# privacy-scaling-explorations/snark-verifier

Hardware: AMD Instinct MI355X
Metric: BN254 G1 MSM points/sec at 2^20 (higher is better)
Workload: dtype i32x9 (254-bit Montgomery Fq as 9 x 29-bit limbs on the integer VALU); 1 GPU; BN254 G1 Pippenger MSM, 2^20 random points/scalars per GPU, inputs resident in HBM, affine result (configs[1]); points_per_gpu=1048576, points_per_kernel_launch=1048576, window_bits=default, msms_in_flight=264

## Files before the change

### snark-verifier_amd/csrc/ctx.hpp

```cpp
#pragma once
#include <hip/hip_runtime.h>
#include <stddef.h>
#include <stdint.h>
#include <stdio.h>
#include "../../include/snarkv_amd.h"
#include "curve_consts.h"

#if defined(SNARKV_CURVE_PALLAS)
#define SNARKV_API(name) snarkv_pallas_##name
#define SNARKV_CHUNK_PIPELINE 0
#define SNARKV_API_FLAGS SNARKV_FLAG_VALIDATE
#else
#define SNARKV_API(name) snarkv_##name
#define SNARKV_CHUNK_PIPELINE 1
#define SNARKV_API_FLAGS (SNARKV_FLAG_VALIDATE | SNARKV_FLAG_MONTGOMERY)
#endif

namespace snarkv {

void set_last_error(const char* fmt, ...);

#define SNARKV_HIP(expr)                                                                   \
  do {                                                                                     \
    hipError_t _e = (expr);                                                                \
    if (_e != hipSuccess) {                                                                \
      ::snarkv::set_last_error("%s:%d: %s -> %s", __FILE__, __LINE__, #expr, hipGetErrorString(_e)); \
      return SNARKV_ERR_DEVICE;                                                            \
    }                                                                                      \
  } while (0)

#define SNARKV_TRY(expr)      \
  do {                        \
    int _rc = (expr);         \
    if (_rc < 0) return _rc;  \
  } while (0)

enum Slot {
  SLOT_IN_SCALARS = 0,
  SLOT_IN_POINTS,
  SLOT_IN_OFFSETS,
  SLOT_OUT,
  SLOT_POINTS_MONT,
  SLOT_COUNTS,
  SLOT_OFFSETS,
  SLOT_CURSOR,
  SLOT_BLOCKSUMS,
  SLOT_ENTRIES,
  SLOT_PIECES,
  SLOT_SPLIT_PARTS,
  SLOT_PIECE_HIST,
  SLOT_BUCKETS,
  SLOT_CHUNK_PARTIALS,
  SLOT_WINDOW_SUMS,
  SLOT_TERM_PARTIALS,
  SLOT_FLAGS,
  SLOT_MISC,
  SLOT_SORT_TMP,
  SLOT_SHIFTED,
  SLOT_GLV,
  SLOT_FIX_LISTS,
  SLOT_MISC2,
  SLOT_TERM_CHAIN,
  SLOT_TERM_MAGS,
  SLOT_SPLIT_PARTIALS,
  SLOT_IPA_XI,
  SLOT_IPA_H,
  SLOT_IPA_OUT,
  SLOT_MGPU_GRID,
  SLOT_MGPU_RECV,
  SLOT_COUNT
};

}

struct snarkv_ctx {
  int device;
  hipStream_t stream;
  bool own_stream;
  void* buf[snarkv::SLOT_COUNT];
  size_t cap[snarkv::SLOT_COUNT];
  void* hbuf[SNARKV_HOST_BUFFERS];
  size_t hbuf_cap[SNARKV_HOST_BUFFERS];
  uint32_t flags;
  bool mont;
  bool stage_timing;
  float stage_ms[SNARKV_PIP_STAGES];
  hipEvent_t ev[SNARKV_PIP_STAGES + 1];
  bool ev_ready;
  snarkv_ctx* sub[4];
  hipEvent_t sub_ev[5];
  bool sub_ready;
  hipEvent_t sorted_ev;
  bool sorted_ev_ready;
  int last_split_workers;
  bool throughput_mode;
  int throughput_peers;
  bool is_lane;
  snarkv_ctx* jobs[SNARKV_MANY_MAX_JOBS];
  int njobs;
  int last_many_jobs;
  size_t many_sig;
  hipStream_t copy_stream;
  bool copy_ready;
  hipEvent_t many_ev[2];
  hipEvent_t order_ev;
  bool order_ev_ready;
  hipStream_t hi_stream[2];
  bool hi_ready;
};

struct snarkv_dk {
  int device;
  void* d_prep;
  uint8_t g1[64];
};

struct snarkv_ipa_dk {
  int device;
  uint32_t k;
  void* d_points;
  size_t first;
  size_t count;
};

namespace snarkv {

struct CallFlags {
  snarkv_ctx* c;
  bool saved;
  CallFlags(snarkv_ctx* ctx, uint32_t call_flags) : c(ctx), saved(ctx ? ctx->mont : false) {
    if (c) c->mont = ((c->flags | call_flags) & SNARKV_FLAG_MONTGOMERY) != 0;
  }
  ~CallFlags() {
    if (c) c->mont = saved;
  }
};
#define SNARKV_CALL_FLAGS(ctx, f) ::snarkv::CallFlags _call_flags((ctx), (f))
struct WireFormScope {
  snarkv_ctx* c;
  bool saved;
  explicit WireFormScope(snarkv_ctx* ctx) : c(ctx), saved(ctx ? ctx->mont : false) {
    if (c) c->mont = false;
// ... 50 lines not shown
```

### snark-verifier_amd/csrc/glv.h

```cpp
#pragma once
#include "fq.h"

namespace snarkv {

template <int NA, int NB, int NOUT>
SNARKV_HD void mp_mul(const uint32_t* a, const uint32_t* b, uint32_t* out) {
#pragma unroll
  for (int i = 0; i < NOUT; ++i) out[i] = 0;
#pragma unroll
  for (int i = 0; i < NA; ++i) {
    uint64_t carry = 0;
#pragma unroll
    for (int j = 0; j < NB; ++j) {
      if (i + j < NOUT) {
        uint64_t t = (uint64_t)a[i] * b[j] + out[i + j] + carry;
        out[i + j] = (uint32_t)t;
        carry = t >> 32;
      }
    }
    if (i + NB < NOUT) out[i + NB] = (uint32_t)carry;
  }
}

SNARKV_HD void glv_decompose(const uint32_t k[8], uint32_t out[8]) {
  constexpr uint32_t A1[4] = SNARKV_GLV_A1;
  constexpr uint32_t NB1[4] = SNARKV_GLV_NEG_B1;
  constexpr uint32_t A2[4] = SNARKV_GLV_A2;
  constexpr uint32_t B2[4] = SNARKV_GLV_B2;
  constexpr uint32_t G1[6] = SNARKV_GLV_G1;
  constexpr uint32_t G2[6] = SNARKV_GLV_G2;
  uint32_t a1[4], nb1[4], a2[4], b2[4], g1[6], g2[6];
  for (int i = 0; i < 4; ++i) { a1[i] = A1[i]; nb1[i] = NB1[i]; a2[i] = A2[i]; b2[i] = B2[i]; }
  for (int i = 0; i < 6; ++i) { g1[i] = G1[i]; g2[i] = G2[i]; }

  uint32_t t1[14], t2[14];
  mp_mul<8, 6, 14>(k, g1, t1);
  mp_mul<8, 6, 14>(k, g2, t2);
  uint32_t c1[5], c2[5];
  {
    uint64_t carry = ((uint64_t)t1[8] + 0x80000000u) >> 32;
    for (int i = 0; i < 5; ++i) {
      uint64_t v = (uint64_t)t1[9 + i] + carry;
      c1[i] = (uint32_t)v;
      carry = v >> 32;
    }
    carry = ((uint64_t)t2[8] + 0x80000000u) >> 32;
    for (int i = 0; i < 5; ++i) {
      uint64_t v = (uint64_t)t2[9 + i] + carry;
      c2[i] = (uint32_t)v;
      carry = v >> 32;
    }
  }
  uint32_t p1[5], p2[5], k1[5], k2[5];
  mp_mul<5, 4, 5>(c1, a1, p1);
  mp_mul<5, 4, 5>(c2, a2, p2);
  {
    uint64_t borrow = 0;
    for (int i = 0; i < 5; ++i) {
      uint64_t v = (uint64_t)k[i] - p1[i] - borrow;
      k1[i] = (uint32_t)v;
      borrow = (v >> 32) & 1u;
    }
    borrow = 0;
    for (int i = 0; i < 5; ++i) {
      uint64_t v = (uint64_t)k1[i] - p2[i] - borrow;
      k1[i] = (uint32_t)v;
      borrow = (v >> 32) & 1u;
    }
  }
  mp_mul<5, 4, 5>(c1, nb1, p1);
  mp_mul<5, 4, 5>(c2, b2, p2);
  {
    uint64_t borrow = 0;
    for (int i = 0; i < 5; ++i) {
      uint64_t v = (uint64_t)p1[i] - p2[i] - borrow;
      k2[i] = (uint32_t)v;
      borrow = (v >> 32) & 1u;
    }
  }
  uint32_t* halves[2] = {k1, k2};
  for (int h = 0; h < 2; ++h) {
    uint32_t* v = halves[h];
    uint32_t neg = v[4] >> 31;
    if (neg) {
      uint64_t carry = 1;
      for (int i = 0; i < 5; ++i) {
        uint64_t x = (uint64_t)(~v[i]) + carry;
        v[i] = (uint32_t)x;
        carry = x >> 32;
      }
    }
    for (int i = 0; i < 4; ++i) out[4 * h + i] = v[i];
    out[4 * h + 3] |= neg << 31;
  }
}

}
```

### snark-verifier_amd/csrc/msm_pippenger.hip

```cpp
#include <stdlib.h>
#include <string.h>
#include <algorithm>
#include <mutex>
#include <atomic>
#include "ctx.hpp"
#include "g1_29.h"
#include "fr29.h"
#ifndef SNARKV_GLV
#define SNARKV_GLV 1
#endif
#if SNARKV_GLV
#include "glv.h"
#endif

namespace snarkv {

#ifndef SNARKV_KRUN
#define SNARKV_KRUN 128
#endif
#ifndef SNARKV_KCHUNK
#define SNARKV_KCHUNK 8
#endif
#ifndef SNARKV_TILE_THREADS
#define SNARKV_TILE_THREADS 256
#endif
#ifndef SNARKV_SCATTER_ATTR
#define SNARKV_SCATTER_ATTR __attribute__((amdgpu_waves_per_eu(5)))
#endif
#ifndef SNARKV_L2_THREADS
#define SNARKV_L2_THREADS 512
#endif
#ifndef SNARKV_LEVEL2_ATTR
#define SNARKV_LEVEL2_ATTR
#endif
#ifndef SNARKV_PREP_THREADS
#define SNARKV_PREP_THREADS SNARKV_TILE_THREADS
#endif
#ifndef SNARKV_XCD_TILES
#define SNARKV_XCD_TILES 1
#endif
#ifndef SNARKV_TILE_BASE
#define SNARKV_TILE_BASE 2048
#endif
#ifndef SNARKV_ACC_WAVES
#define SNARKV_ACC_WAVES 3
#endif
#ifndef SNARKV_BPRIO
#define SNARKV_BPRIO 3
#endif
#define SNARKV_RAISE_PRIO() __builtin_amdgcn_s_setprio(SNARKV_BPRIO)

constexpr int kHalves = SNARKV_GLV ? 2 : 1;
constexpr int kDigitWords = SNARKV_GLV ? 4 : 8;
constexpr int kDigitBits = 32 * kDigitWords;
constexpr int kRun = SNARKV_KRUN;
#ifndef SNARKV_KRUN_THROUGHPUT
#define SNARKV_KRUN_THROUGHPUT 128
#endif
constexpr int kRunThroughput = SNARKV_KRUN_THROUGHPUT;
constexpr int kChunk = SNARKV_KCHUNK;
constexpr uint32_t kSortCap = 7168;
constexpr uint32_t kSortTarget = 3072;
constexpr uint32_t kMaxKeys = 16384;

struct PipParams {
  uint32_t n;
  int c;
  int W;
  uint32_t B;
  uint32_t nb;
  int low_bits;
  uint32_t SB;
  uint32_t nkeys;
  uint32_t nblk;
  uint32_t tile;
  uint32_t mstride;
  uint32_t w0;
  uint32_t krun;
  uint32_t wper;
  uint32_t chunk_log2;
  uint32_t mont;
};

__device__ __forceinline__ uint32_t half_bits(const uint32_t (&k)[kDigitWords], int lo, int c) {
  if (lo >= kDigitBits) return 0;
  int word = lo >> 5, sh = lo & 31;
  uint32_t w0 = 0u, w1 = 0u;
#pragma unroll
  for (int i = 0; i < kDigitWords; ++i) {
    w0 = word == i ? k[i] : w0;
    if (i > 0) w1 = word == i - 1 ? k[i] : w1;
  }
  uint64_t v = ((uint64_t)w1 << 32) | w0;
  return (uint32_t)(v >> sh) & ((1u << c) - 1u);
}

template <class F>
__device__ __forceinline__ void for_each_digit(const uint32_t (&k)[kDigitWords], uint32_t sgn, const PipParams& p, F emit) {
  uint32_t carry = 0;
  for (int w = 0; w < p.W; ++w) {
    uint32_t raw = half_bits(k, w * p.c, p.c) + carry;
    uint32_t neg = raw > p.B ? 1u : 0u;
    uint32_t d = neg ? ((1u << p.c) - raw) : raw;
    carry = neg;
    if (d != 0) emit((uint32_t)w * p.SB + ((d - 1) >> p.low_bits), (uint32_t)w * p.B + d - 1, neg ^ sgn);
  }
}
template <class F>
__device__ __forceinline__ void digit_of_window(const uint32_t (&k)[kDigitWords], uint32_t sgn, const PipParams& p, int w,
                                                F emit) {
  uint32_t carry = 0;
  for (int j = w - 1; j >= 0; --j) {
    uint32_t b = half_bits(k, j * p.c, p.c);
    if (b != p.B) {
      carry = b > p.B ? 1u : 0u;
      break;
    }
  }
  uint32_t raw = half_bits(k, w * p.c, p.c) + carry;
  uint32_t neg = raw > p.B ? 1u : 0u;
  uint32_t d = neg ? ((1u << p.c) - raw) : raw;
  if (d != 0) emit((uint32_t)w * p.SB + ((d - 1) >> p.low_bits), (uint32_t)w * p.B + d - 1, neg ^ sgn);
}
__device__ __forceinline__ uint32_t load_digit_words(const uint32_t* src, uint32_t (&k)[kDigitWords]) {
#pragma unroll
  for (int j = 0; j < kDigitWords; ++j) k[j] = src[j];
#if SNARKV_GLV
  uint32_t sgn = k[3] >> 31;
  k[3] &= 0x7FFFFFFFu;
  return sgn;
#else
  return 0u;
#endif
}
__device__ __forceinline__ uint32_t load_digit_source(const uint4* __restrict__ src, size_t v, uint32_t (&k)[kDigitWords]) {
  const uint4* s = src + v * (kDigitWords / 4);
#pragma unroll
  for (int j = 0; j < kDigitWords / 4; ++j) {
    uint4 q = s[j];
    k[4 * j] = q.x;
    k[4 * j + 1] = q.y;
    k[4 * j + 2] = q.z;
    k[4 * j + 3] = q.w;
  }
#if SNARKV_GLV
  uint32_t sgn = k[3] >> 31;
  k[3] &= 0x7FFFFFFFu;
  return sgn;
#else
  return 0u;
#endif
}

__device__ __forceinline__ uint32_t xcd_tile(uint32_t b, uint32_t nblk) {
#if SNARKV_XCD_TILES
  return (nblk & 7u) == 0 ? (b & 7u) * (nblk >> 3) + (b >> 3) : b;
#else
  return b;
#endif
}

__global__ void __launch_bounds__(SNARKV_PREP_THREADS)
    k_prepare(const uint32_t* __restrict__ scalars, const uint32_t* __restrict__ points,
              G1Packed* __restrict__ pts, uint4* __restrict__ glv, PipParams p, uint32_t* __restrict__ M) {
  SNARKV_RAISE_PRIO();
  extern __shared__ uint32_t lds[];
  for (uint32_t k = threadIdx.x; k < p.nkeys; k += blockDim.x) lds[k] = 0u;
  __syncthreads();
  const uint32_t tile = xcd_tile(blockIdx.x, p.nblk);
  uint32_t lo = tile * p.tile;
  uint32_t hi = lo + p.tile < p.n ? lo + p.tile : p.n;
  for (uint32_t i = lo + threadIdx.x; i < hi; i += blockDim.x) {
    const uint4* s = reinterpret_cast<const uint4*>(points + (size_t)i * 16);
    uint32_t w[16];
#pragma unroll
    for (int j = 0; j < 4; ++j) {
      uint4 v = s[j];
      w[4 * j] = v.x;
      w[4 * j + 1] = v.y;
      w[4 * j + 2] = v.z;
      w[4 * j + 3] = v.w;
    }
    G1Affine29 a = g1a29_from_words(w, p.mont != 0);
    bool ident = g1a29_is_identity(a);
    pts[kHalves * (size_t)i] = g1a29_pack(a);
    const uint4* ks = reinterpret_cast<const uint4*>(scalars + (size_t)i * 8);
    uint4 k0 = ks[0], k1 = ks[1];
    uint32_t k[8] = {k0.x, k0.y, k0.z, k0.w, k1.x, k1.y, k1.z, k1.w}, o[8];
    if (p.mont) {
      uint32_t kc[8];
      fr_words_from_mont256(k, kc);
#pragma unroll
      for (int j = 0; j < 8; ++j) k[j] = kc[j];
    }
#if SNARKV_GLV
    constexpr int32_t bl[9] = SNARKV_GLV_BETA29_LIMBS;
    Fq29 beta;
#pragma unroll
    for (int j = 0; j < 9; ++j) beta.v[j] = bl[j];
    a.x = fq29_canon_of_product(fq29_mul(a.x, beta));
    pts[2 * (size_t)i + 1] = g1a29_pack(a);
    glv_decompose(k, o);
#else
#pragma unroll
    for (int j = 0; j < 8; ++j) o[j] = k[j];
#endif
    if (ident) {
#pragma unroll
      for (int j = 0; j < 8; ++j) o[j] = 0;
    }
    glv[2 * (size_t)i] = make_uint4(o[0], o[1], o[2], o[3]);
    glv[2 * (size_t)i + 1] = make_uint4(o[4], o[5], o[6], o[7]);
#pragma unroll
    for (int h = 0; h < kHalves; ++h) {
      uint32_t d[kDigitWords];
      uint32_t sgn = load_digit_words(o + h * kDigitWords, d);
      for_each_digit(d, sgn, p, [&](uint32_t key, uint32_t, uint32_t) { atomicAdd(&lds[key], 1u); });
    }
  }
  __syncthreads();
  for (uint32_t k = threadIdx.x; k < p.nkeys; k += blockDim.x) M[(size_t)k * p.mstride + tile] = lds[k];
  if (blockIdx.x == 0 && p.mstride > p.nblk)
    for (uint32_t k = threadIdx.x; k < p.nkeys; k += blockDim.x) M[(size_t)k * p.mstride + p.nblk] = 0u;
}

constexpr uint32_t kStageScalars = SNARKV_TILE_BASE;
constexpr uint32_t kStageItems = kStageScalars / SNARKV_TILE_THREADS;
static_assert(kStageScalars % SNARKV_TILE_THREADS == 0, "a staged tile gives every lane the same number of scalars");
__global__ void __launch_bounds__(SNARKV_TILE_THREADS) SNARKV_SCATTER_ATTR
    k_sort_scatter_staged(const uint4* __restrict__ glv, PipParams p, const uint32_t* __restrict__ M,
                          uint2* __restrict__ tmp) {
  SNARKV_RAISE_PRIO();
  extern __shared__ uint32_t lds[];
  uint32_t* gbase = lds;
  uint32_t* cnt = lds + p.SB;
  uint32_t* off = lds + 2 * p.SB;
  uint32_t* wsum = lds + 3 * p.SB;
  uint2* stage = reinterpret_cast<uint2*>(lds + 3 * p.SB + 16 + (p.SB & 1u));
  const uint32_t tid = threadIdx.x, lane = tid & 63u, wave = tid >> 6;
  const uint32_t tile = xcd_tile(blockIdx.x, p.nblk);
  const uint32_t lo = tile * kStageScalars;
  const uint32_t hi = lo + kStageScalars < p.n ? lo + kStageScalars : p.n;
  const uint32_t per = (p.SB + SNARKV_TILE_THREADS - 1) / SNARKV_TILE_THREADS;
  for (int w = 0; w < p.W; ++w) {
    for (uint32_t k = tid; k < p.SB; k += blockDim.x) {
      gbase[k] = M[((size_t)w * p.SB + k) * p.mstride + tile];
      cnt[k] = 0u;
    }
    __syncthreads();
    uint32_t ebkt[kStageItems * kHalves], erank[kStageItems * kHalves], eneg = 0u;
#pragma unroll
    for (uint32_t j = 0; j < kStageItems; ++j) {
      const uint32_t i = lo + tid + j * SNARKV_TILE_THREADS;
#pragma unroll
      for (uint32_t h = 0; h < (uint32_t)kHalves; ++h) {
        const uint32_t e = j * kHalves + h;
        ebkt[e] = 0xFFFFFFFFu;
        if (i < hi) {
          uint32_t d[kDigitWords];
          uint32_t sgn = load_digit_source(glv, (size_t)kHalves * i + h, d);
          digit_of_window(d, sgn, p, w, [&](uint32_t key, uint32_t bucket, uint32_t neg) {
            ebkt[e] = bucket - (uint32_t)w * p.B;
            eneg |= neg << e;
            erank[e] = atomicAdd(&cnt[key - (uint32_t)w * p.SB], 1u);
          });
        }
      }
    }
    __syncthreads();
    uint32_t mine = 0;
    for (uint32_t k = tid * per; k < (tid + 1) * per && k < p.SB; ++k) mine += cnt[k];
    uint32_t incl = mine;
#pragma unroll
    for (int d = 1; d < 64; d <<= 1) {
      uint32_t up = __shfl_up(incl, d, 64);
      if ((int)lane >= d) incl += up;
    }
    if (lane == 63) wsum[wave] = incl;
    __syncthreads();
    uint32_t run = incl - mine;
    for (uint32_t q = 0; q < wave; ++q) run += wsum[q];
    for (uint32_t k = tid * per; k < (tid + 1) * per && k < p.SB; ++k) {
      off[k] = run;
      run += cnt[k];
    }
    __syncthreads();
#pragma unroll
    for (uint32_t e = 0; e < kStageItems * kHalves; ++e)
      if (ebkt[e] != 0xFFFFFFFFu) {
        const uint32_t v = kHalves * (lo + tid + (e / kHalves) * SNARKV_TILE_THREADS) + (e % kHalves);
        stage[off[ebkt[e] >> p.low_bits] + erank[e]] = make_uint2(ebkt[e] + (uint32_t)w * p.B, v | (((eneg >> e) & 1u) << 31));
      }
    __syncthreads();
    const uint32_t total = off[p.SB - 1] + cnt[p.SB - 1];
    for (uint32_t idx = tid; idx < total; idx += blockDim.x) {
      const uint2 e = stage[idx];
      const uint32_t key = (e.x - (uint32_t)w * p.B) >> p.low_bits;
      tmp[gbase[key] + (idx - off[key])] = e;
    }
    __syncthreads();
  }
}

__global__ void __launch_bounds__(256) k_scan_local(uint32_t* __restrict__ data, uint32_t* __restrict__ blocksum,
                                                    uint32_t nb) {
  SNARKV_RAISE_PRIO();
  __shared__ uint32_t sh[256];
  uint32_t base = blockIdx.x * 1024 + threadIdx.x * 4;
  uint32_t v[4], s = 0;
#pragma unroll
  for (int j = 0; j < 4; ++j) {
    v[j] = (base + j < nb) ? data[base + j] : 0;
    s += v[j];
  }
  sh[threadIdx.x] = s;
  __syncthreads();
  for (uint32_t off = 1; off < 256; off <<= 1) {
    uint32_t t = (threadIdx.x >= off) ? sh[threadIdx.x - off] : 0;
    __syncthreads();
    sh[threadIdx.x] += t;
    __syncthreads();
  }
  uint32_t excl = sh[threadIdx.x] - s;
#pragma unroll
  for (int j = 0; j < 4; ++j) {
    if (base + j < nb) data[base + j] = excl;
    excl += v[j];
  }
  if (threadIdx.x == 255) blocksum[blockIdx.x] = sh[255];
}

__global__ void __launch_bounds__(1024) k_scan_blocksums(uint32_t* __restrict__ blocksum, uint32_t nblocks,
                                                         uint32_t* __restrict__ total_out) {
  SNARKV_RAISE_PRIO();
  __shared__ uint32_t sh[1024];
  __shared__ uint32_t running;
  if (threadIdx.x == 0) running = 0;
  __syncthreads();
  for (uint32_t base = 0; base < nblocks; base += 1024) {
    uint32_t idx = base + threadIdx.x;
    uint32_t v = idx < nblocks ? blocksum[idx] : 0;
    sh[threadIdx.x] = v;
    __syncthreads();
    for (uint32_t off = 1; off < 1024; off <<= 1) {
      uint32_t t = (threadIdx.x >= off) ? sh[threadIdx.x - off] : 0;
      __syncthreads();
      sh[threadIdx.x] += t;
      __syncthreads();
    }
    uint32_t r0 = running;
    if (idx < nblocks) blocksum[idx] = r0 + sh[threadIdx.x] - v;
    __syncthreads();
    if (threadIdx.x == 1023) running = r0 + sh[1023];
    __syncthreads();
  }
  if (threadIdx.x == 0) *total_out = running;
}

__global__ void __launch_bounds__(256) k_scan_add(uint32_t* __restrict__ data, const uint32_t* __restrict__ blocksum,
                                                  uint32_t nb) {
  SNARKV_RAISE_PRIO();
  uint32_t base = blockIdx.x * 1024 + threadIdx.x * 4;
  uint32_t add = blocksum[blockIdx.x];
#pragma unroll
  for (int j = 0; j < 4; ++j)
    if (base + j < nb) data[base + j] += add;
}

__global__ void __launch_bounds__(SNARKV_L2_THREADS) SNARKV_LEVEL2_ATTR
    k_sort_level2(const uint2* __restrict__ tmp, const uint32_t* __restrict__ M, uint32_t* __restrict__ misc,
                  PipParams p, uint2* __restrict__ entries, uint32_t* __restrict__ counts,
                  uint32_t* __restrict__ offsets) {
// ... 451 lines not shown
                     (uint32_t*)d_out64, partial_out ? 1 : 0, ctx->mont ? 1u : 0u);
  SNARKV_HIP(hipGetLastError());
  return SNARKV_OK;
}

static int default_window_bits(size_t n) {
  int best = 2;
  double best_cost = 0;
  for (int c = 2; c <= 22; ++c) {
    const int W = (kDigitBits + c - 1) / c;
    const int top = kDigitBits - 1 - (W - 1) * c;
    double cost = (double)kHalves * (double)n * W * 10.0 + (double)W * (double)(1u << (c - 1)) * 30.0;
    if (top < c - 3) cost *= 1.6;
    if (c == 2 || cost < best_cost) best = c, best_cost = cost;
  }
  return best;
}

static int balance_window_bits(int c) {
  int W = (kDigitBits + c - 1) / c;
  return (kDigitBits + W - 1) / W;
}

static uint32_t latency_run_length(uint64_t entries) {
  auto waves = [&](uint64_t run) { return (entries + 64 * run - 1) / (64 * run); };
  if (waves(16) <= 4608) return waves(16) >= 2048 ? 16u : 32u;
  if (waves(32) <= 4608) return 32u;
  return (uint32_t)kRun;
}
static_assert(kRun >= 32 && kRun <= (int)kMaxPiece && kRunThroughput >= 16 && kRunThroughput <= (int)kMaxPiece,
              "piece caps fit the schedule's LDS rows");

int launch_msm_pippenger(snarkv_ctx* ctx, const void* d_scalars, const void* d_points, size_t n, int window_bits,
                         void* d_out, bool partial_out, void* d_buckets_out) {
  return launch_msm_pippenger_phases(ctx, ctx->stream, PIP_PHASE_ALL, d_scalars, d_points, n, window_bits, d_out,
                                     partial_out, d_buckets_out, nullptr);
}

int launch_msm_pippenger_phases(snarkv_ctx* ctx, hipStream_t st, int phases, const void* d_scalars, const void* d_points,
                                size_t n, int window_bits, void* d_out, bool partial_out, void* d_buckets_out,
                                void* d_grid) {
  PipParams p;
  p.w0 = 0;
  p.wper = 0;
  p.chunk_log2 = (uint32_t)kLog2Chunk;
  p.mont = ctx->mont ? 1u : 0u;
  p.n = (uint32_t)n;
  p.c = window_bits > 0 ? window_bits : balance_window_bits(default_window_bits(n));
  if (p.c < 2) p.c = 2;
  if (p.c > 22) p.c = 22;
  p.W = (kDigitBits + p.c - 1) / p.c;
  p.B = 1u << (p.c - 1);
  p.nb = (uint32_t)p.W * p.B;
  int high = p.c - 1 > 10 ? p.c - 1 - 10 : 0;
  while (high < p.c - 1 && ((kHalves * n) >> (high + 1)) >= kSortTarget && ((uint64_t)p.W << (high + 1)) <= kMaxKeys) ++high;
  p.low_bits = (p.c - 1) - high;
  p.SB = p.B >> p.low_bits;
  p.nkeys = (uint32_t)p.W * p.SB;
  p.tile = SNARKV_TILE_BASE;
  static_assert(kStageItems * kHalves <= 32, "a staged lane keeps one sign bit per entry in a 32-bit word");
  const size_t lds_staged = ((size_t)3 * p.SB + 16 + (p.SB & 1u)) * 4 + (size_t)kStageScalars * kHalves * 8;
  p.nblk = (uint32_t)((n + p.tile - 1) / p.tile);
  p.mstride = p.nblk | 1u;
  uint64_t max_entries = (uint64_t)kHalves * (uint64_t)n * (uint64_t)p.W;
  if (n == 0 || max_entries >= 0xFFFFFFFFull || n >= 0x40000000ull) {
    set_last_error("pippenger: n=%zu out of range", n);
    return SNARKV_ERR_LENGTH;
  }
  if ((size_t)p.nkeys * 4 > 65536 || lds_staged > 96 * 1024) {
    set_last_error("pippenger: key table too large (nkeys=%u)", p.nkeys);
    return SNARKV_ERR_LENGTH;
  }
  p.krun = ctx->throughput_mode ? (uint32_t)kRunThroughput : latency_run_length(max_entries);
  const uint32_t max_pieces = (uint32_t)std::min<uint64_t>((uint64_t)p.nb + max_entries / p.krun, 0xFFFFFFFFull - 63);
  const uint32_t split_slots = (uint32_t)(max_entries / p.krun) + 1;
  const uint32_t nsb = (p.nb + kSchedBuckets - 1) / kSchedBuckets;
  const uint32_t hcount = sched_rows(p.krun) * nsb;
  const uint32_t hscan_blocks = (hcount + 1023) / 1024;
  uint32_t mcount = p.nkeys * p.mstride;
  uint32_t scan_blocks = (mcount + 1023) / 1024;
  uint32_t chunks_per_window = (p.B + kChunk - 1) / kChunk;
  uint32_t blocks_per_window = (chunks_per_window + 63) / 64;

  void *d_pts, *d_glv, *d_counts, *d_offsets, *d_M, *d_blocksum, *d_entries, *d_tmp, *d_pieces, *d_hist, *d_parts,
      *d_buckets, *d_wave, *d_shift, *d_misc, *d_lists;
  SNARKV_TRY(ctx_reserve(ctx, SLOT_POINTS_MONT, kHalves * n * sizeof(G1Packed), &d_pts));
  SNARKV_TRY(ctx_reserve(ctx, SLOT_GLV, n * 32, &d_glv));
  SNARKV_TRY(ctx_reserve(ctx, SLOT_COUNTS, (size_t)p.nb * 4, &d_counts));
  SNARKV_TRY(ctx_reserve(ctx, SLOT_OFFSETS, (size_t)p.nb * 4, &d_offsets));
  SNARKV_TRY(ctx_reserve(ctx, SLOT_CURSOR, (size_t)mcount * 4, &d_M));
  SNARKV_TRY(ctx_reserve(ctx, SLOT_BLOCKSUMS, (size_t)std::max(scan_blocks, hscan_blocks) * 4 + 64, &d_blocksum));
  SNARKV_TRY(ctx_reserve(ctx, SLOT_ENTRIES, max_entries * 8, &d_entries));
  SNARKV_TRY(ctx_reserve(ctx, SLOT_SORT_TMP, max_entries * 8, &d_tmp));
  SNARKV_TRY(ctx_reserve(ctx, SLOT_PIECES, (size_t)max_pieces * sizeof(uint4), &d_pieces));
  SNARKV_TRY(ctx_reserve(ctx, SLOT_PIECE_HIST, (size_t)hcount * 4, &d_hist));
  SNARKV_TRY(ctx_reserve(ctx, SLOT_SPLIT_PARTS, (size_t)split_slots * 2 * sizeof(G1Xyzz29), &d_parts));
  if (d_grid) d_buckets = d_grid;
  else SNARKV_TRY(ctx_reserve(ctx, SLOT_BUCKETS, (size_t)p.nb * sizeof(G1Xyzz29), &d_buckets));
  SNARKV_TRY(ctx_reserve(ctx, SLOT_CHUNK_PARTIALS, 2 * (size_t)blocks_per_window * p.W * sizeof(G1Xyzz29), &d_wave));
  SNARKV_TRY(ctx_reserve(ctx, SLOT_SHIFTED, (size_t)p.W * sizeof(G1Xyzz29), &d_shift));
  SNARKV_TRY(ctx_reserve(ctx, SLOT_MISC, 64, &d_misc));
  SNARKV_TRY(ctx_reserve(ctx, SLOT_FIX_LISTS, (size_t)p.nb * 3 * 4, &d_lists));
  uint32_t* d_total = (uint32_t*)d_misc;
  uint32_t* d_small = (uint32_t*)d_lists, *d_bigl = d_small + p.nb, *d_deg = d_bigl + p.nb;
  const uint32_t* d_npieces = (const uint32_t*)d_hist + (size_t)(p.krun + 1) * nsb;

  const bool tm = ctx->stage_timing && phases == PIP_PHASE_ALL;
  const bool tm_acc = ctx->stage_timing && phases == PIP_PHASE_ACC;
  int evi = 0;
#define STAGE_MARK()                                         \
  do {                                                       \
    if (tm) SNARKV_HIP(hipEventRecord(ctx->ev[evi++], st));  \
  } while (0)
  if ((tm || tm_acc) && !ctx->ev_ready) {
    for (int i = 0; i <= SNARKV_PIP_STAGES; ++i) SNARKV_HIP(hipEventCreate(&ctx->ev[i]));
    ctx->ev_ready = true;
  }
  STAGE_MARK();
  if (phases & PIP_PHASE_SORT) {
    hipLaunchKernelGGL(k_prepare, dim3(p.nblk), dim3(SNARKV_PREP_THREADS), (size_t)p.nkeys * 4, st, (const uint32_t*)d_scalars,
                       (const uint32_t*)d_points, (G1Packed*)d_pts, (uint4*)d_glv, p, (uint32_t*)d_M);
    STAGE_MARK();
    hipLaunchKernelGGL(k_scan_local, dim3(scan_blocks), dim3(256), 0, st, (uint32_t*)d_M, (uint32_t*)d_blocksum, mcount);
    hipLaunchKernelGGL(k_scan_blocksums, dim3(1), dim3(1024), 0, st, (uint32_t*)d_blocksum, scan_blocks, d_total);
    hipLaunchKernelGGL(k_scan_add, dim3(scan_blocks), dim3(256), 0, st, (uint32_t*)d_M, (const uint32_t*)d_blocksum,
                       mcount);
    STAGE_MARK();
    static std::atomic<uint64_t> attr_set{0};
    const uint64_t bit = 1ull << (ctx->device & 63);
    if (!(attr_set.load(std::memory_order_relaxed) & bit)) {
      SNARKV_HIP(hipFuncSetAttribute(reinterpret_cast<const void*>(k_sort_scatter_staged),
                                     hipFuncAttributeMaxDynamicSharedMemorySize, 96 * 1024));
      attr_set.fetch_or(bit, std::memory_order_relaxed);
    }
    hipLaunchKernelGGL(k_sort_scatter_staged, dim3(p.nblk), dim3(SNARKV_TILE_THREADS), lds_staged, st, (const uint4*)d_glv,
                       p, (const uint32_t*)d_M, (uint2*)d_tmp);
    const uint32_t nbins_l2 = 1u << p.low_bits;
    const size_t lds2 = ((size_t)nbins_l2 + SNARKV_L2_THREADS + 1) * 4 + (size_t)kSortCap * 8;
    hipLaunchKernelGGL(k_sort_level2, dim3(p.nkeys), dim3(SNARKV_L2_THREADS), lds2, st, (const uint2*)d_tmp, (const uint32_t*)d_M,
                       d_total, p, (uint2*)d_entries, (uint32_t*)d_counts, (uint32_t*)d_offsets);
    hipLaunchKernelGGL(k_piece_hist, dim3(nsb), dim3(256), 0, st, (const uint32_t*)d_counts, p, nsb, (uint32_t*)d_hist,
                       d_total);
    hipLaunchKernelGGL(k_scan_local, dim3(hscan_blocks), dim3(256), 0, st, (uint32_t*)d_hist, (uint32_t*)d_blocksum, hcount);
    hipLaunchKernelGGL(k_scan_blocksums, dim3(1), dim3(1024), 0, st, (uint32_t*)d_blocksum, hscan_blocks, d_total + 6);
    hipLaunchKernelGGL(k_scan_add, dim3(hscan_blocks), dim3(256), 0, st, (uint32_t*)d_hist, (const uint32_t*)d_blocksum,
                       hcount);
    hipLaunchKernelGGL(k_piece_emit, dim3(nsb), dim3(256), 0, st, (const uint32_t*)d_counts, (const uint32_t*)d_offsets, p,
                       nsb, (const uint32_t*)d_hist, split_slots, (uint4*)d_pieces, d_small, d_bigl);
  }
  STAGE_MARK();
  if (tm_acc) SNARKV_HIP(hipEventRecord(ctx->ev[3], st));
  if (phases & PIP_PHASE_ACC)
    hipLaunchKernelGGL(k_accumulate, dim3((max_pieces + 63) / 64), dim3(64), 0, st, (const uint4*)d_pieces, d_npieces,
                       (const uint32_t*)d_total, (const uint2*)d_entries, (const G1Packed*)d_pts, (G1Xyzz29*)d_buckets,
                       (G1Xyzz29*)d_parts, 2 * split_slots, d_total + 4, d_deg, p);
  STAGE_MARK();
  if (tm_acc) SNARKV_HIP(hipEventRecord(ctx->ev[4], st));
  if (phases & PIP_PHASE_ACC) {
    const uint64_t split_bound = std::min<uint64_t>(p.nb, max_entries / (p.krun + 1) + 1);
    const uint32_t fix_grid = (uint32_t)std::min<uint64_t>((split_bound + 255) / 256, kFixGrid);
    hipLaunchKernelGGL(k_fixup, dim3(fix_grid), dim3(256), 0, st, (const uint32_t*)d_counts, (const uint32_t*)d_offsets,
                       (const uint2*)d_entries, (const G1Packed*)d_pts, (const G1Xyzz29*)d_parts, split_slots,
                       (G1Xyzz29*)d_buckets, (const uint32_t*)d_hist, nsb, (const uint32_t*)d_total,
                       (const uint32_t*)d_small, (const uint32_t*)d_bigl, (const uint32_t*)d_deg, p);
    if (tm_acc) SNARKV_HIP(hipEventRecord(ctx->ev[5], st));
  }
  STAGE_MARK();
  if (d_buckets_out) {
    if (phases & PIP_PHASE_ACC)
      SNARKV_HIP(hipMemcpyAsync(d_buckets_out, d_buckets, (size_t)p.nb * sizeof(G1Xyzz29), hipMemcpyDeviceToDevice, st));
    SNARKV_HIP(hipGetLastError());
    return SNARKV_OK;
  }
  if (phases & PIP_PHASE_TAIL)
    hipLaunchKernelGGL(k_bucket_reduce, dim3(blocks_per_window * p.W), dim3(64), 0, st, (const G1Xyzz29*)d_buckets,
                       (G1Xyzz29*)d_wave, p, chunks_per_window, blocks_per_window);
  STAGE_MARK();
  if (phases & PIP_PHASE_TAIL)
    hipLaunchKernelGGL(k_shift_windows, dim3(p.W), dim3(64), 0, st, (const G1Xyzz29*)d_wave, (G1Xyzz29*)d_shift, p,
                       blocks_per_window);
  STAGE_MARK();
  if (phases & PIP_PHASE_TAIL)
    hipLaunchKernelGGL(k_final, dim3(1), dim3(64), 0, st, (const G1Xyzz29*)d_shift, (uint32_t)p.W, (uint32_t*)d_out,
                       partial_out ? 1 : 0, p.mont);
  STAGE_MARK();
#undef STAGE_MARK
  SNARKV_HIP(hipGetLastError());
  return SNARKV_OK;
}

int pip_geometry(size_t n_total, int window_bits, uint32_t* c, uint32_t* windows, uint32_t* buckets_per_window) {
  int cc = window_bits > 0 ? window_bits : balance_window_bits(default_window_bits(n_total));
  if (cc < 2) cc = 2;
  if (cc > 22) cc = 22;
  *c = (uint32_t)cc;
  *windows = (uint32_t)((kDigitBits + cc - 1) / cc);
  *buckets_per_window = 1u << (cc - 1);
  return SNARKV_OK;
}

__global__ void __launch_bounds__(256) k_buckets_add(G1Xyzz29* __restrict__ dst, const G1Xyzz29* __restrict__ src, uint32_t count) {
  SNARKV_RAISE_PRIO();
  uint32_t i = blockIdx.x * blockDim.x + threadIdx.x;
  if (i >= count) return;
  G1Xyzz29 a = dst[i];
  xyzz29_add_careful(a, src[i]);
  dst[i] = xyzz29_sanitize(a);
}

int launch_buckets_add(snarkv_ctx* ctx, void* d_dst, const void* d_src, size_t count) {
  hipLaunchKernelGGL(k_buckets_add, dim3((uint32_t)((count + 255) / 256)), dim3(256), 0, ctx->stream, (G1Xyzz29*)d_dst,
                     (const G1Xyzz29*)d_src, (uint32_t)count);
  SNARKV_HIP(hipGetLastError());
  return SNARKV_OK;
}

int launch_buckets_reduce(snarkv_ctx* ctx, const void* d_buckets, uint32_t c, uint32_t w0, uint32_t wcount,
                          void* d_partial) {
  PipParams p;
// ... 78 lines not shown
```

Measured before the change: 815.5 million points/s.

## Precompute signed window digits in prepare and read them in scatter

The prepare kernel now recodes each GLV half-scalar into signed window digits and writes one packed word per window, laid out window-major. The scatter kernel reads those words directly instead of reloading the 32-byte GLV scalars and recomputing carries by scanning back through lower windows. A specialised path for 16-bit windows extracts digits with shifts only, and the multiprecision multiply is rewritten in column (product-scanning) form. The cost is a larger digit buffer sized to max entries and more HBM writes in prepare, in exchange for cheaper scatter-side reads and less recoding work.

```diff
diff --git a/snark-verifier_amd/csrc/ctx.hpp b/snark-verifier_amd/csrc/ctx.hpp
--- a/snark-verifier_amd/csrc/ctx.hpp
+++ b/snark-verifier_amd/csrc/ctx.hpp
@@ -57,7 +57,7 @@
   SLOT_MISC,
   SLOT_SORT_TMP,
   SLOT_SHIFTED,
-  SLOT_GLV,
+  SLOT_DIGITS,
   SLOT_FIX_LISTS,
   SLOT_MISC2,
   SLOT_TERM_CHAIN,
diff --git a/snark-verifier_amd/csrc/digits.h b/snark-verifier_amd/csrc/digits.h
--- /dev/null
+++ b/snark-verifier_amd/csrc/digits.h
@@ -0,0 +1,64 @@
+#pragma once
+#include "fq.h"
+
+namespace snarkv {
+
+constexpr uint32_t kNoDigit = 0xFFFFFFFFu;
+
+SNARKV_HD uint32_t digit_word(uint32_t bucket, uint32_t neg) { return bucket | (neg << 31); }
+SNARKV_HD bool digit_present(uint32_t word) { return word != kNoDigit; }
+SNARKV_HD uint32_t digit_bucket(uint32_t word) { return word & 0x7FFFFFFFu; }
+SNARKV_HD uint32_t digit_neg(uint32_t word) { return word >> 31; }
+
+template <int NW>
+SNARKV_HD uint32_t half_bits(const uint32_t (&k)[NW], int lo, int c) {
+  if (lo >= 32 * NW) return 0;
+  int word = lo >> 5, sh = lo & 31;
+  uint32_t w0 = 0u, w1 = 0u;
+#pragma unroll
+  for (int i = 0; i < NW; ++i) {
+    w0 = word == i ? k[i] : w0;
+    if (i > 0) w1 = word == i - 1 ? k[i] : w1;
+  }
+  uint64_t v = ((uint64_t)w1 << 32) | w0;
+  return (uint32_t)(v >> sh) & ((1u << c) - 1u);
+}
+
+SNARKV_HD uint32_t recode_window(uint32_t bits, uint32_t& carry, uint32_t sgn, int c) {
+  const uint32_t raw = bits + carry;
+  const uint32_t neg = raw > (1u << (c - 1)) ? 1u : 0u;
+  const uint32_t d = neg ? ((1u << c) - raw) : raw;
+  carry = neg;
+  return d != 0 ? digit_word(d - 1, neg ^ sgn) : kNoDigit;
+}
+
+template <bool C16, int NH, int NW, bool SIGNED, class F>
+SNARKV_HD void for_each_digit(const uint32_t (&src)[NH * NW], int c, int W, F emit) {
+  uint32_t k[NH][NW], sgn[NH], carry[NH];
+#pragma unroll
+  for (int h = 0; h < NH; ++h) {
+#pragma unroll
+    for (int j = 0; j < NW; ++j) k[h][j] = src[h * NW + j];
+    sgn[h] = SIGNED ? k[h][NW - 1] >> 31 : 0u;
+    if (SIGNED) k[h][NW - 1] &= 0x7FFFFFFFu;
+    carry[h] = 0u;
+  }
+  if (C16) {
+#pragma unroll
+    for (int w = 0; w < 2 * NW; ++w) {
+      uint32_t words[NH];
+#pragma unroll
+      for (int h = 0; h < NH; ++h) words[h] = recode_window((k[h][w >> 1] >> (16 * (w & 1))) & 0xFFFFu, carry[h], sgn[h], 16);
+      emit(w, words);
+    }
+  } else {
+    for (int w = 0; w < W; ++w) {
+      uint32_t words[NH];
+#pragma unroll
+      for (int h = 0; h < NH; ++h) words[h] = recode_window(half_bits(k[h], w * c, c), carry[h], sgn[h], c);
+      emit(w, words);
+    }
+  }
+}
+
+}
diff --git a/snark-verifier_amd/csrc/glv.h b/snark-verifier_amd/csrc/glv.h
--- a/snark-verifier_amd/csrc/glv.h
+++ b/snark-verifier_amd/csrc/glv.h
@@ -5,20 +5,22 @@
 
 template <int NA, int NB, int NOUT>
 SNARKV_HD void mp_mul(const uint32_t* a, const uint32_t* b, uint32_t* out) {
+  uint64_t lo = 0;
+  uint32_t hi = 0;
 #pragma unroll
-  for (int i = 0; i < NOUT; ++i) out[i] = 0;
+  for (int k = 0; k < NOUT; ++k) {
 #pragma unroll
-  for (int i = 0; i < NA; ++i) {
-    uint64_t carry = 0;
-#pragma unroll
-    for (int j = 0; j < NB; ++j) {
-      if (i + j < NOUT) {
-        uint64_t t = (uint64_t)a[i] * b[j] + out[i + j] + carry;
-        out[i + j] = (uint32_t)t;
-        carry = t >> 32;
+    for (int i = 0; i < NA; ++i) {
+      const int j = k - i;
+      if (j >= 0 && j < NB) {
+        const uint64_t t = lo + (uint64_t)a[i] * b[j];
+        hi += t < lo ? 1u : 0u;
+        lo = t;
       }
     }
-    if (i + NB < NOUT) out[i + NB] = (uint32_t)carry;
+    out[k] = (uint32_t)lo;
+    lo = (lo >> 32) | ((uint64_t)hi << 32);
+    hi = 0;
   }
 }
 
diff --git a/snark-verifier_amd/csrc/msm_pippenger.hip b/snark-verifier_amd/csrc/msm_pippenger.hip
--- a/snark-verifier_amd/csrc/msm_pippenger.hip
+++ b/snark-verifier_amd/csrc/msm_pippenger.hip
@@ -6,6 +6,7 @@
 #include "ctx.hpp"
 #include "g1_29.h"
 #include "fr29.h"
+#include "digits.h"
 #ifndef SNARKV_GLV
 #define SNARKV_GLV 1
 #endif
@@ -82,76 +83,6 @@
   uint32_t mont;
 };
 
-__device__ __forceinline__ uint32_t half_bits(const uint32_t (&k)[kDigitWords], int lo, int c) {
-  if (lo >= kDigitBits) return 0;
-  int word = lo >> 5, sh = lo & 31;
-  uint32_t w0 = 0u, w1 = 0u;
-#pragma unroll
-  for (int i = 0; i < kDigitWords; ++i) {
-    w0 = word == i ? k[i] : w0;
-    if (i > 0) w1 = word == i - 1 ? k[i] : w1;
-  }
-  uint64_t v = ((uint64_t)w1 << 32) | w0;
-  return (uint32_t)(v >> sh) & ((1u << c) - 1u);
-}
-
-template <class F>
-__device__ __forceinline__ void for_each_digit(const uint32_t (&k)[kDigitWords], uint32_t sgn, const PipParams& p, F emit) {
-  uint32_t carry = 0;
-  for (int w = 0; w < p.W; ++w) {
-    uint32_t raw = half_bits(k, w * p.c, p.c) + carry;
-    uint32_t neg = raw > p.B ? 1u : 0u;
-    uint32_t d = neg ? ((1u << p.c) - raw) : raw;
-    carry = neg;
-    if (d != 0) emit((uint32_t)w * p.SB + ((d - 1) >> p.low_bits), (uint32_t)w * p.B + d - 1, neg ^ sgn);
-  }
-}
-template <class F>
-__device__ __forceinline__ void digit_of_window(const uint32_t (&k)[kDigitWords], uint32_t sgn, const PipParams& p, int w,
-                                                F emit) {
-  uint32_t carry = 0;
-  for (int j = w - 1; j >= 0; --j) {
-    uint32_t b = half_bits(k, j * p.c, p.c);
-    if (b != p.B) {
-      carry = b > p.B ? 1u : 0u;
-      break;
-    }
-  }
-  uint32_t raw = half_bits(k, w * p.c, p.c) + carry;
-  uint32_t neg = raw > p.B ? 1u : 0u;
-  uint32_t d = neg ? ((1u << p.c) - raw) : raw;
-  if (d != 0) emit((uint32_t)w * p.SB + ((d - 1) >> p.low_bits), (uint32_t)w * p.B + d - 1, neg ^ sgn);
-}
-__device__ __forceinline__ uint32_t load_digit_words(const uint32_t* src, uint32_t (&k)[kDigitWords]) {
-#pragma unroll
-  for (int j = 0; j < kDigitWords; ++j) k[j] = src[j];
-#if SNARKV_GLV
-  uint32_t sgn = k[3] >> 31;
-  k[3] &= 0x7FFFFFFFu;
-  return sgn;
-#else
-  return 0u;
-#endif
-}
-__device__ __forceinline__ uint32_t load_digit_source(const uint4* __restrict__ src, size_t v, uint32_t (&k)[kDigitWords]) {
-  const uint4* s = src + v * (kDigitWords / 4);
-#pragma unroll
-  for (int j = 0; j < kDigitWords / 4; ++j) {
-    uint4 q = s[j];
-    k[4 * j] = q.x;
-    k[4 * j + 1] = q.y;
-    k[4 * j + 2] = q.z;
-    k[4 * j + 3] = q.w;
-  }
-#if SNARKV_GLV
-  uint32_t sgn = k[3] >> 31;
-  k[3] &= 0x7FFFFFFFu;
-  return sgn;
-#else
-  return 0u;
-#endif
-}
-
 __device__ __forceinline__ uint32_t xcd_tile(uint32_t b, uint32_t nblk) {
 #if SNARKV_XCD_TILES
   return (nblk & 7u) == 0 ? (b & 7u) * (nblk >> 3) + (b >> 3) : b;
@@ -160,9 +91,10 @@
 #endif
 }
 
+template <bool C16>
 __global__ void __launch_bounds__(SNARKV_PREP_THREADS)
     k_prepare(const uint32_t* __restrict__ scalars, const uint32_t* __restrict__ points,
-              G1Packed* __restrict__ pts, uint4* __restrict__ glv, PipParams p, uint32_t* __restrict__ M) {
+              G1Packed* __restrict__ pts, uint32_t* __restrict__ digits, PipParams p, uint32_t* __restrict__ M) {
   SNARKV_RAISE_PRIO();
   extern __shared__ uint32_t lds[];
   for (uint32_t k = threadIdx.x; k < p.nkeys; k += blockDim.x) lds[k] = 0u;
@@ -209,14 +141,18 @@
 #pragma unroll
       for (int j = 0; j < 8; ++j) o[j] = 0;
     }
-    glv[2 * (size_t)i] = make_uint4(o[0], o[1], o[2], o[3]);
-    glv[2 * (size_t)i + 1] = make_uint4(o[4], o[5], o[6], o[7]);
-#pragma unroll
-    for (int h = 0; h < kHalves; ++h) {
-      uint32_t d[kDigitWords];
-      uint32_t sgn = load_digit_words(o + h * kDigitWords, d);
-      for_each_digit(d, sgn, p, [&](uint32_t key, uint32_t, uint32_t) { atomicAdd(&lds[key], 1u); });
-    }
+    uint32_t* row = digits + (size_t)kHalves * i;
+    for_each_digit<C16, kHalves, kDigitWords, SNARKV_GLV != 0>(o, p.c, p.W, [&](int w, const uint32_t (&word)[kHalves]) {
+      uint32_t* dst = row + (size_t)w * kHalves * p.n;
+#if SNARKV_GLV
+      *reinterpret_cast<uint2*>(dst) = make_uint2(word[0], word[1]);
+#else
+      dst[0] = word[0];
+#endif
+#pragma unroll
+      for (int h = 0; h < kHalves; ++h)
+        if (digit_present(word[h])) atomicAdd(&lds[(uint32_t)w * p.SB + (digit_bucket(word[h]) >> p.low_bits)], 1u);
+    });
   }
   __syncthreads();
   for (uint32_t k = threadIdx.x; k < p.nkeys; k += blockDim.x) M[(size_t)k * p.mstride + tile] = lds[k];
@@ -228,7 +164,7 @@
 constexpr uint32_t kStageItems = kStageScalars / SNARKV_TILE_THREADS;
 static_assert(kStageScalars % SNARKV_TILE_THREADS == 0, "a staged tile gives every lane the same number of scalars");
 __global__ void __launch_bounds__(SNARKV_TILE_THREADS) SNARKV_SCATTER_ATTR
-    k_sort_scatter_staged(const uint4* __restrict__ glv, PipParams p, const uint32_t* __restrict__ M,
+    k_sort_scatter_staged(const uint32_t* __restrict__ digits, PipParams p, const uint32_t* __restrict__ M,
                           uint2* __restrict__ tmp) {
   SNARKV_RAISE_PRIO();
   extern __shared__ uint32_t lds[];
@@ -252,18 +188,26 @@
 #pragma unroll
     for (uint32_t j = 0; j < kStageItems; ++j) {
       const uint32_t i = lo + tid + j * SNARKV_TILE_THREADS;
+      uint32_t word[kHalves];
+#pragma unroll
+      for (int h = 0; h < kHalves; ++h) word[h] = kNoDigit;
+      if (i < hi) {
+        const uint32_t* src = digits + ((size_t)w * p.n + i) * kHalves;
+#if SNARKV_GLV
+        const uint2 q = *reinterpret_cast<const uint2*>(src);
+        word[0] = q.x, word[1] = q.y;
+#else
+        word[0] = src[0];
+#endif
+      }
 #pragma unroll
       for (uint32_t h = 0; h < (uint32_t)kHalves; ++h) {
         const uint32_t e = j * kHalves + h;
-        ebkt[e] = 0xFFFFFFFFu;
-        if (i < hi) {
-          uint32_t d[kDigitWords];
-          uint32_t sgn = load_digit_source(glv, (size_t)kHalves * i + h, d);
-          digit_of_window(d, sgn, p, w, [&](uint32_t key, uint32_t bucket, uint32_t neg) {
-            ebkt[e] = bucket - (uint32_t)w * p.B;
-            eneg |= neg << e;
-            erank[e] = atomicAdd(&cnt[key - (uint32_t)w * p.SB], 1u);
-          });
+        ebkt[e] = kNoDigit;
+        if (digit_present(word[h])) {
+          ebkt[e] = digit_bucket(word[h]);
+          eneg |= digit_neg(word[h]) << e;
+          erank[e] = atomicAdd(&cnt[ebkt[e] >> p.low_bits], 1u);
         }
       }
     }
@@ -287,7 +231,7 @@
     __syncthreads();
 #pragma unroll
     for (uint32_t e = 0; e < kStageItems * kHalves; ++e)
-      if (ebkt[e] != 0xFFFFFFFFu) {
+      if (ebkt[e] != kNoDigit) {
         const uint32_t v = kHalves * (lo + tid + (e / kHalves) * SNARKV_TILE_THREADS) + (e % kHalves);
         stage[off[ebkt[e] >> p.low_bits] + erank[e]] = make_uint2(ebkt[e] + (uint32_t)w * p.B, v | (((eneg >> e) & 1u) << 31));
       }
@@ -905,10 +849,10 @@
   uint32_t chunks_per_window = (p.B + kChunk - 1) / kChunk;
   uint32_t blocks_per_window = (chunks_per_window + 63) / 64;
 
-  void *d_pts, *d_glv, *d_counts, *d_offsets, *d_M, *d_blocksum, *d_entries, *d_tmp, *d_pieces, *d_hist, *d_parts,
+  void *d_pts, *d_digits, *d_counts, *d_offsets, *d_M, *d_blocksum, *d_entries, *d_tmp, *d_pieces, *d_hist, *d_parts,
       *d_buckets, *d_wave, *d_shift, *d_misc, *d_lists;
   SNARKV_TRY(ctx_reserve(ctx, SLOT_POINTS_MONT, kHalves * n * sizeof(G1Packed), &d_pts));
-  SNARKV_TRY(ctx_reserve(ctx, SLOT_GLV, n * 32, &d_glv));
+  SNARKV_TRY(ctx_reserve(ctx, SLOT_DIGITS, max_entries * 4, &d_digits));
   SNARKV_TRY(ctx_reserve(ctx, SLOT_COUNTS, (size_t)p.nb * 4, &d_counts));
   SNARKV_TRY(ctx_reserve(ctx, SLOT_OFFSETS, (size_t)p.nb * 4, &d_offsets));
   SNARKV_TRY(ctx_reserve(ctx, SLOT_CURSOR, (size_t)mcount * 4, &d_M));
@@ -941,8 +885,9 @@
   }
   STAGE_MARK();
   if (phases & PIP_PHASE_SORT) {
-    hipLaunchKernelGGL(k_prepare, dim3(p.nblk), dim3(SNARKV_PREP_THREADS), (size_t)p.nkeys * 4, st, (const uint32_t*)d_scalars,
-                       (const uint32_t*)d_points, (G1Packed*)d_pts, (uint4*)d_glv, p, (uint32_t*)d_M);
+    hipLaunchKernelGGL(p.c == 16 ? k_prepare<true> : k_prepare<false>, dim3(p.nblk), dim3(SNARKV_PREP_THREADS),
+                       (size_t)p.nkeys * 4, st, (const uint32_t*)d_scalars, (const uint32_t*)d_points, (G1Packed*)d_pts,
+                       (uint32_t*)d_digits, p, (uint32_t*)d_M);
     STAGE_MARK();
     hipLaunchKernelGGL(k_scan_local, dim3(scan_blocks), dim3(256), 0, st, (uint32_t*)d_M, (uint32_t*)d_blocksum, mcount);
     hipLaunchKernelGGL(k_scan_blocksums, dim3(1), dim3(1024), 0, st, (uint32_t*)d_blocksum, scan_blocks, d_total);
@@ -956,8 +901,8 @@
                                      hipFuncAttributeMaxDynamicSharedMemorySize, 96 * 1024));
       attr_set.fetch_or(bit, std::memory_order_relaxed);
     }
-    hipLaunchKernelGGL(k_sort_scatter_staged, dim3(p.nblk), dim3(SNARKV_TILE_THREADS), lds_staged, st, (const uint4*)d_glv,
-                       p, (const uint32_t*)d_M, (uint2*)d_tmp);
+    hipLaunchKernelGGL(k_sort_scatter_staged, dim3(p.nblk), dim3(SNARKV_TILE_THREADS), lds_staged, st,
+                       (const uint32_t*)d_digits, p, (const uint32_t*)d_M, (uint2*)d_tmp);
     const uint32_t nbins_l2 = 1u << p.low_bits;
     const size_t lds2 = ((size_t)nbins_l2 + SNARKV_L2_THREADS + 1) * 4 + (size_t)kSortCap * 8;
     hipLaunchKernelGGL(k_sort_level2, dim3(p.nkeys), dim3(SNARKV_L2_THREADS), lds2, st, (const uint2*)d_tmp, (const uint32_t*)d_M,
```

After: 820.8 million points/s, median of 6. Within noise of the previous version (+0.6%).
